# tmoroney/whisper-diarize-rs

Hardware: AMD Instinct MI355X
Metric: audio-sec/wall-sec (xRT), large-v3 + DTW + diarize, 1/2/4/8 MI355X (higher is better)
Workload: dtype f16 (f32 accumulate)

## Files before the change

whisper-diarize-rs_amd/csrc/kernels/gemm.hip:

```cpp
#include "../common.h"
#include "../prof.h"

#include <algorithm>
#include <cstdlib>

namespace wdr {

typedef _Float16 f16x2 __attribute__((ext_vector_type(2)));

constexpr int GB_M = 128, GB_N = 128, GB_K = 32;
constexpr int GLDS = GB_K + 8;

template <int EPI>
__device__ __forceinline__ void epi_store(const ProjArgs& a, int row, int col, float v) {
  if (row >= a.M || col >= a.N) return;
  if (a.bias) v += a.bias[col];
  if constexpr (EPI == EPI_F16) {
    ((f16*)a.out)[(size_t)row * a.ldo + col] = (f16)v;
  } else if constexpr (EPI == EPI_F16_GELU) {
    ((f16*)a.out)[(size_t)row * a.ldo + col] = (f16)gelu_tanh(v);
  } else if constexpr (EPI == EPI_F32_RESID) {
    float* o = (float*)a.out + (size_t)row * a.ldo + col;
    *o = *o + v;
  } else if constexpr (EPI == EPI_F32) {
// ... 962 lines not shown
  const __amdgpu_buffer_rsrc_t rsb = __builtin_amdgcn_make_buffer_rsrc((void*)a.b_sc, (short)0, nk * a.ld_bsc * 4, 0x00020000);
  const uint32_t offs = (uint32_t)lane * 16u;
  auto stage_sc = [&](int kt) {
    uint8_t* dst = sc_lds + (kt % 3) * 2048;
    if (wid == 0)
      __builtin_amdgcn_raw_ptr_buffer_load_lds(rsa, (lds_ptr)dst, 16, offs, (kt * a.ld_asc + bm * G3_M) * 4, 0, 0);
    else if (wid == 1 && lane < 32)
      __builtin_amdgcn_raw_ptr_buffer_load_lds(rsb, (lds_ptr)(dst + 1024), 16, offs, (kt * a.ld_bsc + bn * 128) * 4, 0, 0);
  };
  stage_sc(0);
  stage(0, 0, 0);
  stage(0, 2, 0);
  stage(0, 1, 0);
  if (nk > 1) {
    stage_sc(1);
    stage(1, 0, G8_BK);
    stage(1, 2, G8_BK);
    asm volatile("s_waitcnt vmcnt(6)" ::: "memory");
  } else {
    asm volatile("s_waitcnt vmcnt(2)" ::: "memory");
  }
  __builtin_amdgcn_s_barrier();
  if (grp == 1) __builtin_amdgcn_s_barrier();
  __builtin_amdgcn_sched_barrier(0);

  f32x4 acc[8][2];
#pragma unroll
  for (int i = 0; i < 8; ++i)
#pragma unroll
    for (int j = 0; j < 2; ++j) acc[i][j] = f32x4{0.f, 0.f, 0.f, 0.f};

  const int fr = lane & 15, fq = lane >> 4;
  i32x8 af[4], bf[2];
  int sa[4], sb[2];
  auto frag = [&](const uint8_t* img, int r) {
    const i32x4 lo = lds_read16(img + r * 128 + g2_swz(r, fq) * 16);
    const i32x4 hi = lds_read16(img + r * 128 + g2_swz(r, 4 + fq) * 16);
    return (i32x8)__builtin_shufflevector(lo, hi, 0, 1, 2, 3, 4, 5, 6, 7);
  };
  auto read_a = [&](const uint8_t* img, const uint32_t* sc, int h) {
#pragma unroll
    for (int i = 0; i < 4; ++i) {
      af[i] = frag(img, grp * 64 + i * 16 + fr);
      sa[i] = (int)(lds_read4(sc + grp * 128 + 64 * h + i * 16 + fr) >> (8 * fq));
    }
  };
  auto read_b = [&](const uint8_t* img, const uint32_t* sc) {
#pragma unroll
    for (int j = 0; j < 2; ++j) {
      bf[j] = frag(img, wn * 32 + j * 16 + fr);
      sb[j] = (int)(lds_read4(sc + 256 + wn * 32 + j * 16 + fr) >> (8 * fq));
    }
  };
  auto mfma_h = [&](int h) {
    __builtin_amdgcn_s_setprio(1);
#pragma unroll
    for (int i = 0; i < 4; ++i)
#pragma unroll
      for (int j = 0; j < 2; ++j)
        acc[h * 4 + i][j] = __builtin_amdgcn_mfma_scale_f32_16x16x128_f8f6f4(bf[j], af[i], acc[h * 4 + i][j], 0, 0, 0,
                                                                             sb[j], 0, sa[i]);
#pragma unroll
    for (int i = 0; i < 4; ++i) asm volatile("" : "+v"(acc[h * 4 + i][0]), "+v"(acc[h * 4 + i][1]));
    __builtin_amdgcn_s_setprio(0);
  };
  auto sync_in = [&]() {
    asm volatile("s_waitcnt lgkmcnt(0)" ::: "memory");
    __builtin_amdgcn_sched_barrier(0);
    __builtin_amdgcn_s_barrier();
    __builtin_amdgcn_sched_barrier(0);
  };
  auto sync_out = [&]() {
    __builtin_amdgcn_sched_barrier(0);
    __builtin_amdgcn_s_barrier();
    __builtin_amdgcn_sched_barrier(0);
  };

  for (int kt = 0; kt < nk; ++kt) {
    const int cur = kt & 1;
    const uint8_t* img = lds + cur * 3 * HB;
    const uint32_t* sc = (const uint32_t*)(sc_lds + (kt % 3) * 2048);
    const bool n1 = kt + 1 < nk, n2 = kt + 2 < nk;
    read_b(img + 2 * HB, sc);
    read_a(img, sc, 0);
    if (n1) {
      stage(cur ^ 1, 1, (kt + 1) * G8_BK);
      asm volatile("s_waitcnt vmcnt(6)" ::: "memory");
    } else {
      asm volatile("s_waitcnt vmcnt(0)" ::: "memory");
    }
    sync_in();
    mfma_h(0);
    sync_out();
    read_a(img + HB, sc, 1);
    if (n2) {
      stage_sc(kt + 2);
      stage(cur, 0, (kt + 2) * G8_BK);
      stage(cur, 2, (kt + 2) * G8_BK);
      asm volatile("s_waitcnt vmcnt(6)" ::: "memory");
    } else if (n1) {
      asm volatile("s_waitcnt vmcnt(2)" ::: "memory");
    } else {
      asm volatile("s_waitcnt vmcnt(0)" ::: "memory");
    }
    sync_in();
    mfma_h(1);
    sync_out();
  }
  if (grp == 0) __builtin_amdgcn_s_barrier();

  const bool hb = a.bias != nullptr;
  f32x4 bz[2];
#pragma unroll
  for (int j = 0; j < 2; ++j)
    bz[j] = hb ? *(const f32x4*)(a.bias + bn * 128 + wn * 32 + j * 16 + fq * 4) : f32x4{0.f, 0.f, 0.f, 0.f};
#pragma unroll
  for (int i = 0; i < 8; ++i)
#pragma unroll
    for (int j = 0; j < 2; ++j)
      epi_store4<EPI>(a, bm * G3_M + grp * 128 + i * 16 + fr, bn * 128 + wn * 32 + j * 16 + fq * 4, acc[i][j], hb, bz[j]);
}

template <int EPI>
__global__ __launch_bounds__(512, 1) void k_gemm8n(ProjArgs a) {
  ProfClock prof_clock_(a.ts);
  extern __shared__ __attribute__((aligned(16))) uint8_t lds8n[];
  const int ntiles = (a.N / 128) * cdiv(a.M, G3_M);
  for (int t = blockIdx.x; t < ntiles; t += gridDim.x) {
    gemm8n_tile<EPI>(a, lds8n, t, ntiles);
    __builtin_amdgcn_s_barrier();
  }
}

template <int EPI>
static void launch_epi8(const ProjArgs& a, hipStream_t s) {
  const double ob = EPI == EPI_F8_GELU ? 1.0 : (EPI == EPI_F32_RESID || EPI == EPI_F32) ? 4.0 : 2.0;
  const double bytes = ((double)a.N + a.M) * a.K * (1.0 + 1.0 / 32) + (double)a.M * a.N * ob;
  const double flops = 2.0 * a.M * a.N * a.K;
  static bool attr = [] {
    WDR_HIP(hipFuncSetAttribute((const void*)k_gemm8<EPI>, hipFuncAttributeMaxDynamicSharedMemorySize, (int)G8_LDS));
    return true;
  }();
  (void)attr;
  static const int tile_gm = getenv("WDR_GEMM4_GM") ? atoi(getenv("WDR_GEMM4_GM")) : 4;
  ProjArgs g = a;
  g.tile_gm = tile_gm;
  if constexpr (EPI != EPI_F8_GELU) {
    static const bool narrow_on = !getenv("WDR_GEMM8N") || atoi(getenv("WDR_GEMM8N")) != 0;
    if ((narrow_on && a.N < 2048) || a.N % G3_N != 0) {
      static bool attrn = [] {
        WDR_HIP(hipFuncSetAttribute((const void*)k_gemm8n<EPI>, hipFuncAttributeMaxDynamicSharedMemorySize, (int)G8N_LDS));
        return true;
      }();
      (void)attrn;
      const int ntn = (a.N / 128) * cdiv(a.M, G3_M);
      wdr_launch(PROF_GEMM, bytes, flops, k_gemm8n<EPI>, dim3(ntn), dim3(512), G8N_LDS, s, g);
      return;
    }
  }
  const int ntiles = (a.N / G3_N) * cdiv(a.M, G3_M);
  wdr_launch(PROF_GEMM, bytes, flops, k_gemm8<EPI>, dim3(ntiles), dim3(512), G8_LDS, s, g);
}

void launch_proj_fp8(const ProjArgs& a, hipStream_t s) {
  WDR_CHECK(a.A8 && a.B8 && a.a_sc && a.b_sc, "fp8 projection: operands / scales missing");
  WDR_CHECK(a.M > 64 && a.N % 128 == 0 && (a.epi != EPI_F8_GELU || a.N % G3_N == 0) && a.K % G8_BK == 0 &&
                a.lda % 16 == 0 && a.ldb % 16 == 0,
            "fp8 projection: M > 64, N % 128 == 0 (N % 256 for the GELU -> fp8 epilogue), K % 128 == 0, "
            "lda / ldb % 16 required");
  WDR_CHECK(a.ld_asc >= cdiv(a.M, G3_M) * G3_M && a.ld_bsc >= a.N && a.ld_asc % 4 == 0 && a.ld_bsc % 4 == 0,
            "fp8 projection: scale images need the rows rounded up to 256");
  WDR_CHECK(a.epi != EPI_F8_GELU || (a.o_sc && a.ld_osc >= cdiv(a.M, G3_M) * G3_M && a.ldo % 16 == 0),
            "fp8 projection: GELU -> fp8 epilogue needs an output scale image");
  switch (a.epi) {
    case EPI_F16: launch_epi8<EPI_F16>(a, s); break;
    case EPI_F16_GELU: launch_epi8<EPI_F16_GELU>(a, s); break;
    case EPI_F32_RESID: launch_epi8<EPI_F32_RESID>(a, s); break;
    case EPI_F32: launch_epi8<EPI_F32>(a, s); break;
    case EPI_F8_GELU: launch_epi8<EPI_F8_GELU>(a, s); break;
    default: throw std::runtime_error("fp8 projection: unsupported epilogue");
  }
  WDR_HIP(hipGetLastError());
}

__global__ __launch_bounds__(256) void k_quant_f8(const f16* x, int ldx, int rows, int K, uint8_t* y, int ldy,
                                                  uint32_t* sc, int ld_sc) {
  const int row = blockIdx.x * 4 + (threadIdx.x >> 6), lane = threadIdx.x & 63;
  if (row >= rows) return;
  const f16* xr = x + (size_t)row * ldx;
  for (int c0 = 0; c0 < K; c0 += 512) {
    const int c = c0 + lane * 8;
    const bool ok = c < K;
    f16x8 v = ok ? *(const f16x8*)(xr + c) : f16x8{};
    float am = 0.f;
#pragma unroll
    for (int e = 0; e < 8; ++e) am = fmaxf(am, fabsf((float)v[e]));
    am = fmaxf(am, __shfl_xor(am, 1, 64));
    am = fmaxf(am, __shfl_xor(am, 2, 64));
    const int e = f8_block_exp(am);
    const float inv = f8_pow2(-e);
    const uint32_t lo = f8_pack4((float)v[0] * inv, (float)v[1] * inv, (float)v[2] * inv, (float)v[3] * inv);
    const uint32_t hi = f8_pack4((float)v[4] * inv, (float)v[5] * inv, (float)v[6] * inv, (float)v[7] * inv);
    if (ok) *(uint2*)(y + (size_t)row * ldy + c) = make_uint2(lo, hi);
    const int b = e + 127, base = lane & ~15;
    const uint32_t w = (uint32_t)__shfl(b, base, 64) | (uint32_t)__shfl(b, base + 4, 64) << 8 |
                       (uint32_t)__shfl(b, base + 8, 64) << 16 | (uint32_t)__shfl(b, base + 12, 64) << 24;
    if ((lane & 15) == 0 && ok) sc[(size_t)(c >> 7) * ld_sc + row] = w;
  }
}

__global__ __launch_bounds__(64) void k_probe_mfma_scale(const i32x8* a, const i32x8* b, const int* sa, const int* sb,
                                                          f32x4* out) {
  const int l = threadIdx.x;
  out[l] = __builtin_amdgcn_mfma_scale_f32_16x16x128_f8f6f4(a[l], b[l], f32x4{0.f, 0.f, 0.f, 0.f}, 0, 0, 0, sa[l], 0,
                                                             sb[l]);
}
void launch_probe_mfma_scale(const void* a, const void* b, const int* sa, const int* sb, float* out, hipStream_t s) {
  WDR_KLAUNCH(k_probe_mfma_scale, dim3(1), dim3(64), 0, s, (const i32x8*)a, (const i32x8*)b, sa, sb, (f32x4*)out);
  WDR_HIP(hipGetLastError());
}

void launch_quant_f8(const f16* x, int ldx, int rows, int K, uint8_t* y, int ldy, uint32_t* sc, int ld_sc,
                     hipStream_t s) {
  WDR_CHECK(rows >= 1 && K % 128 == 0 && ldx % 8 == 0 && ldy % 16 == 0 && ld_sc >= rows,
            "fp8 quantisation: K % 128, ldx % 8, ldy % 16, scale rows");
  WDR_KLAUNCH(k_quant_f8, dim3(cdiv(rows, 4)), dim3(256), 0, s, x, ldx, rows, K, y, ldy, sc, ld_sc);
  WDR_HIP(hipGetLastError());
}

__global__ __launch_bounds__(256) void k_layernorm_f8(const float* x, int ldx, const float* g, const float* b,
                                                      uint8_t* y, int ldy, uint32_t* sc, int ld_sc, int rows, int d) {
  const int row = blockIdx.x * 4 + (threadIdx.x >> 6);
  const int lane = threadIdx.x & 63;
  if (row >= rows) return;
  const float* xr = x + (long long)row * ldx;
  float v[5][4];
  float s = 0.f;
#pragma unroll
  for (int j = 0; j < 5; ++j) {
    const int c = lane * 4 + j * 256;
    const bool ok = c < d;
    const int cc = ok ? c : 0;
    const float4 q = *(const float4*)(xr + cc);
    v[j][0] = ok ? q.x : 0.f; v[j][1] = ok ? q.y : 0.f; v[j][2] = ok ? q.z : 0.f; v[j][3] = ok ? q.w : 0.f;
    s += (v[j][0] + v[j][1]) + (v[j][2] + v[j][3]);
  }
  s = wave_sum(s);
  const float mean = s / d;
  float s2 = 0.f;
#pragma unroll
  for (int j = 0; j < 5; ++j)
    if (lane * 4 + j * 256 < d)
#pragma unroll
      for (int e = 0; e < 4; ++e) {
        const float t = v[j][e] - mean;
        s2 += t * t;
      }
  s2 = wave_sum(s2);
  const float scale = 1.0f / sqrtf(s2 / d + 1e-5f);
#pragma unroll
  for (int j = 0; j < 5; ++j) {
    const int c = lane * 4 + j * 256;
    if (j * 256 >= d) break;
    const bool ok = c < d;
    const int cc = ok ? c : 0;
    const float4 g4 = *(const float4*)(g + cc);
    const float4 b4 = *(const float4*)(b + cc);
    const float gg[4] = {g4.x, g4.y, g4.z, g4.w}, bb[4] = {b4.x, b4.y, b4.z, b4.w};
    float o[4], am = 0.f;
#pragma unroll
    for (int e = 0; e < 4; ++e) {
      o[e] = ok ? (v[j][e] - mean) * scale * gg[e] + bb[e] : 0.f;
      am = fmaxf(am, fabsf(o[e]));
    }
    am = fmaxf(am, __shfl_xor(am, 1, 64));
    am = fmaxf(am, __shfl_xor(am, 2, 64));
    am = fmaxf(am, __shfl_xor(am, 4, 64));
    const int e = f8_block_exp(am);
    const float inv = f8_pow2(-e);
    if (ok) *(uint32_t*)(y + (size_t)row * ldy + c) = f8_pack4(o[0] * inv, o[1] * inv, o[2] * inv, o[3] * inv);
    const int bb8 = e + 127, base = lane & 32;
    const uint32_t w = (uint32_t)__shfl(bb8, base, 64) | (uint32_t)__shfl(bb8, base + 8, 64) << 8 |
                       (uint32_t)__shfl(bb8, base + 16, 64) << 16 | (uint32_t)__shfl(bb8, base + 24, 64) << 24;
    if ((lane & 31) == 0 && ok) sc[(size_t)(c >> 7) * ld_sc + row] = w;
  }
}

void launch_layernorm_f8(const float* x, int ldx, const float* g, const float* b, uint8_t* y, int ldy, uint32_t* sc,
                         int ld_sc, int rows, int d, hipStream_t s) {
  WDR_CHECK(d % 128 == 0 && d <= 1280 && ldx % 4 == 0 && ldy % 16 == 0 && ld_sc >= rows,
            "fp8 layernorm: d % 128, d <= 1280");
  WDR_KLAUNCH(k_layernorm_f8, dim3(cdiv(rows, 4)), dim3(256), 0, s, x, ldx, g, b, y, ldy, sc, ld_sc, rows, d);
  WDR_HIP(hipGetLastError());
}

template <int EPI, int MT, int NT, int W>
constexpr uint32_t skinny_red_bytes() { return (uint32_t)W * MT * NT * 4 * 64 * 4; }
template <int EPI, int MT, int NT, int W>
static uint32_t skinny_ln_lds(int K) {
  return std::max((uint32_t)16 * MT * K * 2, skinny_red_bytes<EPI, MT, NT, W>());
}

template <int EPI, int MT, int NT, int W = 4, bool LN = false, int UU = 0>
__global__ __launch_bounds__(W * 64) void k_skinny(ProjArgs a) {
  ProfClock prof_clock_(a.ts);
  __shared__ float red_s[LN ? 1 : W * MT * NT * 4 * 64];
  extern __shared__ __attribute__((aligned(16))) f16 xln[];
  float* red = LN ? (float*)xln : red_s;
  const int lane = threadIdx.x & 63, wid = threadIdx.x >> 6;
  const int n0 = blockIdx.x * 16 * NT;
  const int m0 = blockIdx.y * 16 * MT;
  const int fr = lane & 15, fk = 8 * (lane >> 4);
  f32x4 acc[MT][NT];
#pragma unroll
  for (int i = 0; i < MT; ++i)
#pragma unroll
    for (int j = 0; j < NT; ++j) acc[i][j] = (f32x4){0.f, 0.f, 0.f, 0.f};
  const int lds_ld = a.K;
  if constexpr (LN) {
    const int d = a.K;
    const int live = min(16 * MT, a.M - m0);
    for (int rr = wid; rr < live; rr += W) {
      int row = m0 + rr;
      if (a.row_map) row = a.row_map[row];
      const float* xr = a.ln_x + (long long)row * a.ldln;
      float v[5][4];
      float sm = 0.f;
#pragma unroll
      for (int j = 0; j < 5; ++j) {
        const int c = lane * 4 + j * 256;
        const bool ok = c < d;
        const int cc = ok ? c : 0;
        const float4 q = *(const float4*)(xr + cc);
        v[j][0] = ok ? q.x : 0.f; v[j][1] = ok ? q.y : 0.f; v[j][2] = ok ? q.z : 0.f; v[j][3] = ok ? q.w : 0.f;
        sm += (v[j][0] + v[j][1]) + (v[j][2] + v[j][3]);
      }
      sm = wave_sum(sm);
      const float mean = sm / d;
      float s2 = 0.f;
#pragma unroll
      for (int j = 0; j < 5; ++j)
        if (lane * 4 + j * 256 < d)
#pragma unroll
          for (int e = 0; e < 4; ++e) {
            const float t = v[j][e] - mean;
            s2 += t * t;
          }
      s2 = wave_sum(s2);
      const float scale = 1.0f / sqrtf(s2 / d + 1e-5f);
#pragma unroll
      for (int j = 0; j < 5; ++j) {
        const int c = lane * 4 + j * 256;
        if (c >= d) continue;
        const float4 g4 = *(const float4*)(a.ln_g + c);
        const float4 b4 = *(const float4*)(a.ln_b + c);
        const float gg[4] = {g4.x, g4.y, g4.z, g4.w}, bb[4] = {b4.x, b4.y, b4.z, b4.w};
        f16x4 o;
#pragma unroll
        for (int e = 0; e < 4; ++e) o[e] = (f16)((v[j][e] - mean) * scale * gg[e] + bb[e]);
        *(f16x4*)(xln + rr * lds_ld + ((((c >> 3) ^ (rr & 15))) << 3) + (c & 7)) = o;
      }
    }
    __syncthreads();
  }
  const f16* arow[MT];
#pragma unroll
  for (int i = 0; i < MT; ++i) {
    int m = m0 + i * 16 + fr;
    m = m < a.M ? m : a.M - 1;
    if (!LN && a.row_map) m = a.row_map[m];
    arow[i] = LN ? xln + (i * 16 + fr) * lds_ld : a.A + (size_t)m * a.lda + fk;
  }
  const f16* brow[NT];
#pragma unroll
  for (int j = 0; j < NT; ++j) {
    int n = n0 + j * 16 + fr;
    n = n < a.N ? n : a.N - 1;
    brow[j] = a.B + (size_t)n * a.ldb + fk;
  }
  constexpr int U = UU > 0 ? UU : (MT + NT) <= 3 ? 8 : 4;
  for (int k0 = wid * 32; k0 < a.K; k0 += 32 * W * U) {
    f16x8 bf[U][NT], af[U][MT];
#pragma unroll
    for (int u = 0; u < U; ++u) {
      const int k = k0 + u * 32 * W;
      const bool ok = k < a.K;
      const int kk = ok ? k : 0;
#pragma unroll
      for (int j = 0; j < NT; ++j) {
        const f16x8 t = *(const f16x8*)(brow[j] + kk);
        bf[u][j] = ok ? t : (f16x8){};
      }
#pragma unroll
      for (int i = 0; i < MT; ++i) {
        const f16x8 t = LN ? *(const f16x8*)(arow[i] + ((((kk >> 3) | (lane >> 4)) ^ fr) << 3))
                           : *(const f16x8*)(arow[i] + kk);
        af[u][i] = ok ? t : (f16x8){};
      }
    }
#pragma unroll
    for (int u = 0; u < U; ++u)
#pragma unroll
      for (int i = 0; i < MT; ++i)
#pragma unroll
        for (int j = 0; j < NT; ++j)
          acc[i][j] = __builtin_amdgcn_mfma_f32_16x16x32_f16(af[u][i], bf[u][j], acc[i][j], 0, 0, 0);
  }
  if constexpr (LN) __syncthreads();
#pragma unroll
  for (int i = 0; i < MT; ++i)
#pragma unroll
    for (int j = 0; j < NT; ++j)
#pragma unroll
      for (int r = 0; r < 4; ++r) red[(((wid * MT + i) * NT + j) * 4 + r) * 64 + lane] = acc[i][j][r];
  __syncthreads();
  for (int e = threadIdx.x; e < MT * NT * 4 * 64; e += W * 64) {
    const int l = e & 63, r = (e >> 6) & 3, j = (e >> 8) % NT, i = (e >> 8) / NT;
    float v = 0.f;
#pragma unroll
    for (int w = 0; w < W; ++w) v += red[(((w * MT + i) * NT + j) * 4 + r) * 64 + l];
    const int row = m0 + i * 16 + (l >> 4) * 4 + r, col = n0 + j * 16 + (l & 15);
    epi_store<EPI>(a, row, col, v);
  }
}



struct GemmKnobs {
  bool gemm1, gemm3, gemm5, gemm5w;
  int gemm4, tile_gm, cus;
};
static int env_int(const char* name, int def) {
  const char* e = getenv(name);
  return e ? atoi(e) : def;
}
static GemmKnobs read_knobs() {
  GemmKnobs k;
  k.gemm1 = env_int("WDR_GEMM1", 0) != 0;
  k.gemm3 = env_int("WDR_GEMM3", 1) != 0 && !k.gemm1;
  k.gemm4 = env_int("WDR_GEMM4", -1);
  k.tile_gm = env_int("WDR_GEMM4_GM", 4);
  k.gemm5 = env_int("WDR_GEMM5", 0) != 0;
  k.gemm5w = env_int("WDR_GEMM5_WIDE", 1) != 0;
  k.cus = env_int("WDR_GEMM_CUS", 0) / 8 * 8;
  return k;
}
static GemmKnobs& knobs() {
  static GemmKnobs k = read_knobs();
  return k;
}
void gemm_knobs_reload() { knobs() = read_knobs(); }

template <int EPI>
static void launch_epi(const ProjArgs& a, hipStream_t s) {
  const int ob = (EPI == EPI_F32_RESID || EPI == EPI_F32 || EPI == EPI_F32_GELU_POS) ? 4 : 2;
  const double bytes = (double)a.N * a.K * 2 + (double)a.M * a.K * 2 + (double)a.M * a.N * ob;
  const double flops = 2.0 * a.M * a.N * a.K;
  WDR_CHECK(a.M > 64, "encoder GEMM: more than 64 rows (fewer go to the row kernel)");
  const GemmKnobs& kn = knobs();
  const bool ref = kn.gemm1 || a.gemm_ref;
  const bool vec4 = a.ldo % 4 == 0 && (a.epi != EPI_QKV_CACHE || a.d % 4 == 0);
  const bool wide5 = kn.gemm5w && a.N >= 4096 && a.N < 16384 && a.M >= 4096;
  if (a.N % 128 == 0 && a.K % G3_BK == 0 && a.M >= 4096 && !ref && vec4 && kn.gemm4 != 0 &&
      (wide5 || (a.N < 2048 && kn.gemm5 && (a.N / G3_N) * cdiv(a.M, G3_M) < 192))) {
    static bool attr5 = [] {
      WDR_HIP(hipFuncSetAttribute((const void*)k_gemm5<EPI>, hipFuncAttributeMaxDynamicSharedMemorySize, (int)G5_LDS));
      return true;
    }();
    (void)attr5;
    ProjArgs g = a;
    g.tile_gm = kn.tile_gm;
    const int ntiles5 = (a.N / 128) * cdiv(a.M, G3_M);
    dim3 grid(kn.cus > 0 && kn.cus < ntiles5 ? kn.cus : ntiles5);
    wdr_launch(PROF_GEMM, bytes, flops, k_gemm5<EPI>, grid, dim3(512), G5_LDS, s, g);
  } else if (a.N % G3_N == 0 && a.K % G3_BK == 0 && !ref && vec4 &&
             (kn.gemm4 == 1 ||
              (kn.gemm4 != 0 && (a.M >= 4096 || a.N >= 16384 || (a.N >= 4096 && a.M > 1024) ||
                                 (a.N >= 3072 && a.M >= 2560))))) {
    static bool attr4 = [] {
      WDR_HIP(hipFuncSetAttribute((const void*)k_gemm4<EPI>, hipFuncAttributeMaxDynamicSharedMemorySize, (int)G4_LDS));
      return true;
    }();
    (void)attr4;
    const int ntiles = (a.N / G3_N) * cdiv(a.M, G3_M);
    dim3 grid(kn.cus > 0 && kn.cus < ntiles ? kn.cus : ntiles);
    ProjArgs g = a;
    g.tile_gm = kn.tile_gm;
    wdr_launch(PROF_GEMM, bytes, flops, k_gemm4<EPI>, grid, dim3(512), G4_LDS, s, g);
  } else if ((a.N >= 5120 || a.M >= 9000) && a.M > 2048 && a.N % G3_N == 0 && a.K % G3_BK == 0 && kn.gemm3 && !ref) {
    static bool attr = [] {
      WDR_HIP(hipFuncSetAttribute((const void*)k_gemm3<EPI>, hipFuncAttributeMaxDynamicSharedMemorySize, (int)G3_LDS));
      return true;
    }();
    (void)attr;
    dim3 grid((a.N / G3_N) * cdiv(a.M, G3_M));
    wdr_launch(PROF_GEMM, bytes, flops, k_gemm3<EPI>, grid, dim3(512), G3_LDS, s, a);
  } else if (a.K % G2_BK == 0 && a.N <= 4096 && !ref && vec4) {
    dim3 grid((a.N / GB_N) * cdiv(a.M, GB_M));
    wdr_launch(PROF_GEMM, bytes, flops, k_gemm2<EPI>, grid, dim3(256), 0, s, a);
  } else {
    dim3 grid(a.N / GB_N, cdiv(a.M, GB_M));
    wdr_launch(PROF_GEMM, bytes, flops, k_gemm<EPI>, grid, dim3(256), 0, s, a);
  }
}

static bool rows_pair_tiles() {
  static const bool v = env_int("WDR_ROWS_PAIR", 1) != 0;
  return v;
}
static int rows_mt_max() {
  static const int v = std::max(2, std::min(5, env_int("WDR_ROWS_MT", 2)));
  return v;
}

template <int EPI>
static void launch_rows_epi(const ProjArgs& a, hipStream_t s) {
  const double bytes = (double)a.N * a.K * 2;
  const double flops = 2.0 * a.M * a.N * a.K;
  const int mt = cdiv(a.M, 16);
  const bool ln = a.ln_x != nullptr;
  const bool wide = a.N >= 4096;
  const int prof = PROF_GEMV;
  if (!wide) {
    if (a.K > 2048) {
      WDR_CHECK(!ln, "row projection: LN prologue needs K <= 1280");
      if (mt >= 4 && rows_pair_tiles()) {
        const int m2 = std::min(mt, rows_mt_max());
        const dim3 g2(cdiv(a.N, 16), cdiv(mt, m2));
        if (m2 >= 4) wdr_launch(prof, bytes, flops, k_skinny<EPI, 4, 1, 16, false, 2>, g2, dim3(1024), 0, s, a);
        else if (m2 == 3) wdr_launch(prof, bytes, flops, k_skinny<EPI, 3, 1, 16, false, 5>, g2, dim3(1024), 0, s, a);
        else wdr_launch(prof, bytes, flops, k_skinny<EPI, 2, 1, 16, false, 5>, g2, dim3(1024), 0, s, a);
        return;
      }
      wdr_launch(prof, bytes, flops, k_skinny<EPI, 1, 1, 16, false, 12>, dim3(cdiv(a.N, 16), mt), dim3(1024), 0, s, a);
      return;
    }
    if (!ln && mt > 2 && rows_pair_tiles()) {
      const int m2 = std::min(mt, rows_mt_max());
      const dim3 g2(cdiv(a.N, 16), cdiv(mt, m2));
      if (m2 >= 5) wdr_launch(prof, bytes, flops, k_skinny<EPI, 5, 1, 8>, g2, dim3(512), 0, s, a);
      else if (m2 == 4) wdr_launch(prof, bytes, flops, k_skinny<EPI, 4, 1, 8>, g2, dim3(512), 0, s, a);
      else if (m2 == 3) wdr_launch(prof, bytes, flops, k_skinny<EPI, 3, 1, 8>, g2, dim3(512), 0, s, a);
      else wdr_launch(prof, bytes, flops, k_skinny<EPI, 2, 1, 8>, g2, dim3(512), 0, s, a);
      return;
    }
    dim3 grid(cdiv(a.N, 16), mt), blk(512);
    if (ln) wdr_launch(prof, bytes, flops, k_skinny<EPI, 1, 1, 8, true>, grid, blk, skinny_ln_lds<EPI, 1, 1, 8>(a.K), s, a);
    else wdr_launch(prof, bytes, flops, k_skinny<EPI, 1, 1, 8>, grid, blk, 0, s, a);
    return;
  }
  const int mtw = std::min(mt, ln ? 2 : 4);
  dim3 grid(cdiv(a.N, 32), cdiv(mt, mtw)), blk(512);
#define WDR_RW(MTV)                                                                                        \
  if (ln) wdr_launch(prof, bytes, flops, k_skinny<EPI, MTV, 2, 8, true>, grid, blk, skinny_ln_lds<EPI, MTV, 2, 8>(a.K), s, a); \
  else wdr_launch(prof, bytes, flops, k_skinny<EPI, MTV, 2, 8>, grid, blk, 0, s, a);
  if (mtw == 1) { WDR_RW(1) }
  else if (mtw == 2) { WDR_RW(2) }
  else if (mtw == 3) { WDR_RW(3) }
  else { WDR_RW(4) }
#undef WDR_RW
}

static void launch_rows(const ProjArgs& a, hipStream_t s) {
  WDR_CHECK(a.K % 32 == 0 && a.lda % 8 == 0 && a.ldb % 8 == 0, "row projection: K % 32, lda / ldb % 8");
  WDR_CHECK(!a.ln_x || (a.K <= 1280 && a.K % 128 == 0), "row projection LN prologue: K <= 1280, K % 128 == 0");
  WDR_CHECK(a.epi != EPI_QKV_CACHE || (a.kc && a.vc && a.row_seq && a.row_pos && a.d > 0), "qkv-cache epilogue args");
  switch (a.epi) {
    case EPI_F16: launch_rows_epi<EPI_F16>(a, s); break;
    case EPI_F16_GELU: launch_rows_epi<EPI_F16_GELU>(a, s); break;
    case EPI_F32_RESID: launch_rows_epi<EPI_F32_RESID>(a, s); break;
    case EPI_F32: launch_rows_epi<EPI_F32>(a, s); break;
    case EPI_QKV_CACHE: launch_rows_epi<EPI_QKV_CACHE>(a, s); break;
    default: throw std::runtime_error("row projection: bad epilogue");
  }
  WDR_HIP(hipGetLastError());
}

void launch_proj(const ProjArgs& a, hipStream_t s) {
  WDR_CHECK(a.M > 0 && a.K > 0 && a.N > 0, "projection: empty shape");
  if (a.rows_mma || a.M <= 64) {
    launch_rows(a, s);
    return;
  }
  WDR_CHECK(a.K % 8 == 0 && a.lda % 8 == 0 && a.ldb % 8 == 0, "projection: K/lda/ldb must be multiples of 8");
  WDR_CHECK(a.N % GB_N == 0, "gemm: N must be a multiple of 128");
  WDR_CHECK(a.K % GB_K == 0, "gemm: K must be a multiple of 32");
  WDR_CHECK(a.epi != EPI_QKV_CACHE || (a.kc && a.vc && a.row_seq && a.row_pos && a.d > 0), "qkv-cache epilogue args");
  switch (a.epi) {
    case EPI_F16: launch_epi<EPI_F16>(a, s); break;
    case EPI_F16_GELU: launch_epi<EPI_F16_GELU>(a, s); break;
    case EPI_F32_RESID: launch_epi<EPI_F32_RESID>(a, s); break;
    case EPI_F32: launch_epi<EPI_F32>(a, s); break;
    case EPI_F32_GELU_POS: launch_epi<EPI_F32_GELU_POS>(a, s); break;
    case EPI_QKV_CACHE: launch_epi<EPI_QKV_CACHE>(a, s); break;
    case EPI_XKV:
      WDR_CHECK(a.M > 64 && a.seq_stride > 0, "cross-K/V epilogue: encoder GEMM rows and a slot stride");
      launch_epi<EPI_XKV>(a, s);
      break;
    default: throw std::runtime_error("projection: bad epilogue");
  }
  WDR_HIP(hipGetLastError());
}

}
```

Before: 881.1.

## Prefetch weights during LN prologue and add wider LN-fused skinny GEMM tiles

In the LayerNorm-fused skinny decoder GEMM, the first batch of weight fragments is now loaded before the LN prologue, so weight fetch latency overlaps the row normalization. The LN prologue processes two rows per wave together to add memory-level parallelism. New tile shapes (2x2, and 2x4 for wide N) are used for LN projections with more rows, with an occupancy launch bound and a raised dynamic-LDS attribute. The cost is higher register pressure and more dispatch branches, which could lower occupancy on some shapes.

```diff
diff --git a/whisper-diarize-rs_amd/csrc/kernels/gemm.hip b/whisper-diarize-rs_amd/csrc/kernels/gemm.hip
--- a/whisper-diarize-rs_amd/csrc/kernels/gemm.hip
+++ b/whisper-diarize-rs_amd/csrc/kernels/gemm.hip
@@ -1288,11 +1288,14 @@
 }
 
 template <int EPI, int MT, int NT, int W = 4, bool LN = false, int UU = 0>
-__global__ __launch_bounds__(W * 64) void k_skinny(ProjArgs a) {
+__global__ __launch_bounds__(W * 64, (LN && MT <= 2) ? 4 : 1) void k_skinny(ProjArgs a) {
   ProfClock prof_clock_(a.ts);
-  __shared__ float red_s[LN ? 1 : W * MT * NT * 4 * 64];
   extern __shared__ __attribute__((aligned(16))) f16 xln[];
-  float* red = LN ? (float*)xln : red_s;
+  float* red = (float*)xln;
+  if constexpr (!LN) {
+    __shared__ float red_s[W * MT * NT * 4 * 64];
+    red = red_s;
+  }
   const int lane = threadIdx.x & 63, wid = threadIdx.x >> 6;
   const int n0 = blockIdx.x * 16 * NT;
   const int m0 = blockIdx.y * 16 * MT;
@@ -1303,48 +1306,84 @@
 #pragma unroll
     for (int j = 0; j < NT; ++j) acc[i][j] = (f32x4){0.f, 0.f, 0.f, 0.f};
   const int lds_ld = a.K;
+  const f16* brow[NT];
+#pragma unroll
+  for (int j = 0; j < NT; ++j) {
+    int n = n0 + j * 16 + fr;
+    n = n < a.N ? n : a.N - 1;
+    brow[j] = a.B + (size_t)n * a.ldb + fk;
+  }
+  constexpr int U = UU > 0 ? UU : (MT + NT) <= 3 ? 8 : 4;
+  f16x8 bpre[LN ? U : 1][NT];
+  auto load_b = [&](int k0, f16x8(&bf)[LN ? U : 1][NT]) {
+#pragma unroll
+    for (int u = 0; u < (LN ? U : 1); ++u) {
+      const int k = k0 + u * 32 * W;
+      const bool ok = k < a.K;
+      const int kk = ok ? k : 0;
+#pragma unroll
+      for (int j = 0; j < NT; ++j) {
+        const f16x8 t = *(const f16x8*)(brow[j] + kk);
+        bf[u][j] = ok ? t : (f16x8){};
+      }
+    }
+  };
   if constexpr (LN) {
+    load_b(wid * 32, bpre);
     const int d = a.K;
     const int live = min(16 * MT, a.M - m0);
-    for (int rr = wid; rr < live; rr += W) {
-      int row = m0 + rr;
-      if (a.row_map) row = a.row_map[row];
-      const float* xr = a.ln_x + (long long)row * a.ldln;
-      float v[5][4];
-      float sm = 0.f;
-#pragma unroll
-      for (int j = 0; j < 5; ++j) {
-        const int c = lane * 4 + j * 256;
-        const bool ok = c < d;
-        const int cc = ok ? c : 0;
-        const float4 q = *(const float4*)(xr + cc);
-        v[j][0] = ok ? q.x : 0.f; v[j][1] = ok ? q.y : 0.f; v[j][2] = ok ? q.z : 0.f; v[j][3] = ok ? q.w : 0.f;
-        sm += (v[j][0] + v[j][1]) + (v[j][2] + v[j][3]);
-      }
-      sm = wave_sum(sm);
-      const float mean = sm / d;
-      float s2 = 0.f;
-#pragma unroll
-      for (int j = 0; j < 5; ++j)
-        if (lane * 4 + j * 256 < d)
-#pragma unroll
-          for (int e = 0; e < 4; ++e) {
-            const float t = v[j][e] - mean;
-            s2 += t * t;
-          }
-      s2 = wave_sum(s2);
-      const float scale = 1.0f / sqrtf(s2 / d + 1e-5f);
-#pragma unroll
-      for (int j = 0; j < 5; ++j) {
-        const int c = lane * 4 + j * 256;
-        if (c >= d) continue;
-        const float4 g4 = *(const float4*)(a.ln_g + c);
-        const float4 b4 = *(const float4*)(a.ln_b + c);
-        const float gg[4] = {g4.x, g4.y, g4.z, g4.w}, bb[4] = {b4.x, b4.y, b4.z, b4.w};
-        f16x4 o;
-#pragma unroll
-        for (int e = 0; e < 4; ++e) o[e] = (f16)((v[j][e] - mean) * scale * gg[e] + bb[e]);
-        *(f16x4*)(xln + rr * lds_ld + ((((c >> 3) ^ (rr & 15))) << 3) + (c & 7)) = o;
+    constexpr int RPW = 16 * MT / W, RB = (MT == 1 && NT == 2) ? 1 : 2;
+    static_assert(16 * MT % W == 0 && RPW % RB == 0, "LN prologue: whole batches of rows per wave");
+    for (int b0 = 0; b0 < RPW; b0 += RB) {
+      if (wid + b0 * W >= live) break;
+      float v[RB][5][4];
+#pragma unroll
+      for (int i = 0; i < RB; ++i) {
+        const int rr = wid + (b0 + i) * W;
+        int row = m0 + (rr < live ? rr : live - 1);
+        if (a.row_map) row = a.row_map[row];
+        const float* xr = a.ln_x + (long long)row * a.ldln;
+#pragma unroll
+        for (int j = 0; j < 5; ++j) {
+          const int c = lane * 4 + j * 256;
+          const bool ok = c < d;
+          const int cc = ok ? c : 0;
+          const float4 q = *(const float4*)(xr + cc);
+          v[i][j][0] = ok ? q.x : 0.f; v[i][j][1] = ok ? q.y : 0.f; v[i][j][2] = ok ? q.z : 0.f; v[i][j][3] = ok ? q.w : 0.f;
+        }
+      }
+#pragma unroll
+      for (int i = 0; i < RB; ++i) {
+        const int rr = wid + (b0 + i) * W;
+        if (rr >= live) break;
+        float sm = 0.f;
+#pragma unroll
+        for (int j = 0; j < 5; ++j) sm += (v[i][j][0] + v[i][j][1]) + (v[i][j][2] + v[i][j][3]);
+        sm = wave_sum(sm);
+        const float mean = sm / d;
+        float s2 = 0.f;
+#pragma unroll
+        for (int j = 0; j < 5; ++j)
+          if (lane * 4 + j * 256 < d)
+#pragma unroll
+            for (int e = 0; e < 4; ++e) {
+              const float t = v[i][j][e] - mean;
+              s2 += t * t;
+            }
+        s2 = wave_sum(s2);
+        const float scale = 1.0f / sqrtf(s2 / d + 1e-5f);
+#pragma unroll
+        for (int j = 0; j < 5; ++j) {
+          const int c = lane * 4 + j * 256;
+          if (c >= d) continue;
+          const float4 g4 = *(const float4*)(a.ln_g + c);
+          const float4 b4 = *(const float4*)(a.ln_b + c);
+          const float gg[4] = {g4.x, g4.y, g4.z, g4.w}, bb[4] = {b4.x, b4.y, b4.z, b4.w};
+          f16x4 o;
+#pragma unroll
+          for (int e = 0; e < 4; ++e) o[e] = (f16)((v[i][j][e] - mean) * scale * gg[e] + bb[e]);
+          *(f16x4*)(xln + rr * lds_ld + ((((c >> 3) ^ (rr & 15))) << 3) + (c & 7)) = o;
+        }
       }
     }
     __syncthreads();
@@ -1357,15 +1396,31 @@
     if (!LN && a.row_map) m = a.row_map[m];
     arow[i] = LN ? xln + (i * 16 + fr) * lds_ld : a.A + (size_t)m * a.lda + fk;
   }
-  const f16* brow[NT];
-#pragma unroll
-  for (int j = 0; j < NT; ++j) {
-    int n = n0 + j * 16 + fr;
-    n = n < a.N ? n : a.N - 1;
-    brow[j] = a.B + (size_t)n * a.ldb + fk;
-  }
-  constexpr int U = UU > 0 ? UU : (MT + NT) <= 3 ? 8 : 4;
-  for (int k0 = wid * 32; k0 < a.K; k0 += 32 * W * U) {
+  if constexpr (LN) {
+    for (int k0 = wid * 32; k0 < a.K; k0 += 32 * W * U) {
+      if (k0 != wid * 32) load_b(k0, bpre);
+      f16x8 af[U][MT];
+#pragma unroll
+      for (int u = 0; u < U; ++u) {
+        const int k = k0 + u * 32 * W;
+        const bool ok = k < a.K;
+        const int kk = ok ? k : 0;
+#pragma unroll
+        for (int i = 0; i < MT; ++i) {
+          const f16x8 t = *(const f16x8*)(arow[i] + ((((kk >> 3) | (lane >> 4)) ^ fr) << 3));
+          af[u][i] = ok ? t : (f16x8){};
+        }
+      }
+#pragma unroll
+      for (int u = 0; u < U; ++u)
+#pragma unroll
+        for (int i = 0; i < MT; ++i)
+#pragma unroll
+          for (int j = 0; j < NT; ++j)
+            acc[i][j] = __builtin_amdgcn_mfma_f32_16x16x32_f16(af[u][i], bpre[u][j], acc[i][j], 0, 0, 0);
+    }
+  }
+  for (int k0 = wid * 32; !LN && k0 < a.K; k0 += 32 * W * U) {
     f16x8 bf[U][NT], af[U][MT];
 #pragma unroll
     for (int u = 0; u < U; ++u) {
@@ -1499,6 +1554,18 @@
   return v;
 }
 
+template <int EPI, int MT, int NT, int UU = 0>
+static void launch_skinny_ln(const ProjArgs& a, dim3 grid, double bytes, double flops, hipStream_t s) {
+  static bool attr = [] {
+    WDR_HIP(hipFuncSetAttribute((const void*)k_skinny<EPI, MT, NT, 8, true, UU>,
+                                hipFuncAttributeMaxDynamicSharedMemorySize, (int)skinny_ln_lds<EPI, MT, NT, 8>(1280)));
+    return true;
+  }();
+  (void)attr;
+  wdr_launch(PROF_GEMV, bytes, flops, k_skinny<EPI, MT, NT, 8, true, UU>, grid, dim3(512),
+             skinny_ln_lds<EPI, MT, NT, 8>(a.K), s, a);
+}
+
 template <int EPI>
 static void launch_rows_epi(const ProjArgs& a, hipStream_t s) {
   const double bytes = (double)a.N * a.K * 2;
@@ -1521,6 +1588,10 @@
       wdr_launch(prof, bytes, flops, k_skinny<EPI, 1, 1, 16, false, 12>, dim3(cdiv(a.N, 16), mt), dim3(1024), 0, s, a);
       return;
     }
+    if (ln && mt > 2 && rows_pair_tiles() && cdiv(a.N, 16) * mt > 320) {
+      launch_skinny_ln<EPI, 2, 2>(a, dim3(cdiv(a.N, 32), cdiv(mt, 2)), bytes, flops, s);
+      return;
+    }
     if (!ln && mt > 2 && rows_pair_tiles()) {
       const int m2 = std::min(mt, rows_mt_max());
       const dim3 g2(cdiv(a.N, 16), cdiv(mt, m2));
@@ -1531,19 +1602,23 @@
       return;
     }
     dim3 grid(cdiv(a.N, 16), mt), blk(512);
-    if (ln) wdr_launch(prof, bytes, flops, k_skinny<EPI, 1, 1, 8, true>, grid, blk, skinny_ln_lds<EPI, 1, 1, 8>(a.K), s, a);
+    if (ln) launch_skinny_ln<EPI, 1, 1>(a, grid, bytes, flops, s);
     else wdr_launch(prof, bytes, flops, k_skinny<EPI, 1, 1, 8>, grid, blk, 0, s, a);
     return;
   }
+  if (ln && mt > 5) {
+    launch_skinny_ln<EPI, 2, 4, 2>(a, dim3(cdiv(a.N, 64), cdiv(mt, 2)), bytes, flops, s);
+    return;
+  }
   const int mtw = std::min(mt, ln ? 2 : 4);
   dim3 grid(cdiv(a.N, 32), cdiv(mt, mtw)), blk(512);
-#define WDR_RW(MTV)                                                                                        \
-  if (ln) wdr_launch(prof, bytes, flops, k_skinny<EPI, MTV, 2, 8, true>, grid, blk, skinny_ln_lds<EPI, MTV, 2, 8>(a.K), s, a); \
+#define WDR_RW(MTV)                                                             \
+  if (ln) launch_skinny_ln<EPI, MTV, 2>(a, grid, bytes, flops, s);              \
   else wdr_launch(prof, bytes, flops, k_skinny<EPI, MTV, 2, 8>, grid, blk, 0, s, a);
   if (mtw == 1) { WDR_RW(1) }
   else if (mtw == 2) { WDR_RW(2) }
-  else if (mtw == 3) { WDR_RW(3) }
-  else { WDR_RW(4) }
+  else if (mtw == 3) wdr_launch(prof, bytes, flops, k_skinny<EPI, 3, 2, 8>, grid, blk, 0, s, a);
+  else wdr_launch(prof, bytes, flops, k_skinny<EPI, 4, 2, 8>, grid, blk, 0, s, a);
 #undef WDR_RW
 }
 
```

Measured after the change: 878.8. About the same (-0.3%).
